# D-Hank/NeRF-tiny

Hardware: AMD Instinct MI355X
Metric: rays/sec (64 coarse + 128 fine samples), lego 400x400 (higher is better)
Workload: dtype f32

## Files before the change

### nerf-tiny_amd/csrc/field_fwd_reg.hip

```cpp
#include "field_common.h"
#include <type_traits>

namespace nerf {

constexpr int RM = 32;

template <int I0, int I1, class F>
__device__ __forceinline__ void static_for(F&& f) {
  if constexpr (I0 < I1) {
    f(std::integral_constant<int, I0>{});
    static_for<I0 + 1, I1>(f);
  }
}

template <int NFT>
struct WStage {
  float4 w[NFT];
};

template <int KB, int NFT>
__device__ __forceinline__ void stage_load(const float4* __restrict__ seg_lane, int kb, WStage<NFT>& s) {
#pragma unroll
  for (int f = 0; f < NFT; ++f) s.w[f] = seg_lane[(size_t)(f * KB + kb) * 64];
}

__device__ __forceinline__ float relu1(float x) { return __int_as_float(max(__float_as_int(x), 0)); }

__device__ __forceinline__ float f4c(const float4& v, int c) { return c == 0 ? v.x : (c == 1 ? v.y : (c == 2 ? v.z : v.w)); }

typedef int lds_i32 __attribute__((address_space(3), may_alias));
typedef int i32x4v __attribute__((ext_vector_type(4), may_alias));
typedef __attribute__((address_space(3))) i32x4v lds_i32x4;
constexpr int RELU_LDS_DWORDS = 2 * 4 * 64 * 4;
constexpr int COL_LDS_DWORDS = 3 * HALF + 4;
struct ReluLds {
  lds_i32* w;
  lds_i32* m[4];
};
__device__ __forceinline__ ReluLds relu_lds(lds_i32* base, int lane) {
  ReluLds L;
  L.w = base + 4 * lane;
#pragma unroll
  for (int c = 0; c < 4; ++c) L.m[c] = base + 4 * lane + ((c + (lane >> 3)) & 3);
  return L;
}
__device__ __forceinline__ float4 lds_ld4(const lds_i32* p) {
  const i32x4v v = *reinterpret_cast<const lds_i32x4*>(p);
  return make_float4(__int_as_float(v[0]), __int_as_float(v[1]), __int_as_float(v[2]), __int_as_float(v[3]));
}
template <typename DST>
__device__ __forceinline__ void relu_lds_op(const ReluLds& L, const f32x16& src, DST& dst, int dst0, int slot, int i) {
  const int g = i / 6, j = i - 6 * g, off = (slot * 4 + g) * 256;
  if (j == 0) {
    const i32x4v v = {__float_as_int(src[4 * g]), __float_as_int(src[4 * g + 1]), __float_as_int(src[4 * g + 2]), __float_as_int(src[4 * g + 3])};
    *reinterpret_cast<lds_i32x4*>(L.w + off) = v;
  } else if (j < 5) {
    __hip_atomic_fetch_max(L.m[j - 1] + off, 0, __ATOMIC_RELAXED, __HIP_MEMORY_SCOPE_WORKGROUP);
  } else {
    const i32x4v v = *reinterpret_cast<lds_i32x4*>(L.w + off);
#pragma unroll
    for (int c = 0; c < 4; ++c) dst[dst0 + c] = __int_as_float(v[c]);
  }
}

struct SaveIn {
  float* rows;
  uint16_t* mask;
};

__device__ __forceinline__ void bias_group(const float* b4h, int t, int g, f32x16& acc) {
  const float4 q = *reinterpret_cast<const float4*>(b4h + 32 * t + 8 * g);
  acc[4 * g + 0] = q.x;
  acc[4 * g + 1] = q.y;
  acc[4 * g + 2] = q.z;
  acc[4 * g + 3] = q.w;
}

template <int KB, int NFT, int NKB, int NNFT, bool ZERO_INIT, bool RELU_IN, int SAVE = 0, bool LDS_RELU = false, bool NEXT_RELU = false, int NEXT_BIAS = 0>
__device__ __forceinline__ void reg_layer(const int seg, const int next_seg , int lane,
                                          const f32x16* prev, f32x16* acc, WStage<8>& st0, const float* bv,
                                          const SaveIn sv, const RegBuf& rb, const ReluLds& rl, f32x4v& head,
                                          const float* nb = nullptr, f32x16* nacc = nullptr) {
  static_assert(!(LDS_RELU || NEXT_RELU || NEXT_BIAS) || SAVE != 1, "the saving forward keeps the VALU ReLU and the bias MFMAs");
  static_assert(NEXT_BIAS == 0 || ((LDS_RELU && RELU_IN) || NEXT_RELU), "the bias loads live in the stream with compile-time k-blocks");
  static_assert(NEXT_BIAS != 1 || (KB == 32 && RELU_IN), "NEXT_BIAS = 1 overwrites the 8 input tiles of a 256-wide ReLU layer");
  static_assert(NEXT_BIAS != 2 || KB == 8, "NEXT_BIAS = 2: one tile per k-block of layer 0");
  constexpr int KT = KB / 4;
  constexpr bool LR = LDS_RELU && RELU_IN;
  WStage<8> st1;
  const f32x16 zero = {0.f, 0.f, 0.f, 0.f, 0.f, 0.f, 0.f, 0.f, 0.f, 0.f, 0.f, 0.f, 0.f, 0.f, 0.f, 0.f};
  if (bv != nullptr) {
    const float one_h0 = (lane < 32) ? 1.0f : 0.0f;
#pragma unroll
    for (int f = 0; f < NFT; ++f) acc[f] = __builtin_amdgcn_mfma_f32_32x32x2f32(bv[f], one_h0, zero, 0, 0, 0);
  }
  f32x16 tin[2];
  if constexpr (LR) {
#pragma unroll
    for (int c = 0; c < 4; ++c) tin[0][c] = head[c];
    if (bv != nullptr) {
#pragma unroll
      for (int i = 6; i < 14; ++i) relu_lds_op(rl, prev[0], tin[0], 4 * (i / 6), 0, i);
#pragma unroll
      for (int i = 6; i < 14; ++i) {
        __builtin_amdgcn_sched_group_barrier(0x008, 1, 0);
        __builtin_amdgcn_sched_group_barrier(0x080, 1, 0);
      }
    }
  }
  [[maybe_unused]] const int lr0 = (bv != nullptr) ? 14 : 6;
  auto mask_word = [&](int t) {
    unsigned bits = 0;
#pragma unroll
    for (int r = 0; r < 16; ++r) bits |= (prev[t][r] > 0.f) ? (1u << r) : 0u;
    sv.mask[((t & 1) * 2) * 256 + (t >> 1) * 64] = (uint16_t)bits;
  };
  auto activate = [&](int t) {
    if constexpr (LR) {
      if (SAVE != 0) mask_word(t);
      return;
    }
#pragma unroll
    for (int r = 0; r < 16; ++r) tin[t & 1][r] = RELU_IN ? (SAVE == 1 ? fmaxf(prev[t][r], 0.f) : relu1(prev[t][r])) : prev[t][r];
#pragma unroll
    for (int r = 0; r < 16; ++r) asm volatile("" : "+v"(tin[t & 1][r]));
    if (SAVE == 1 || (SAVE == 2 && !RELU_IN)) {
#pragma unroll
      for (int g = 0; g < 4; ++g)
        store_row4(sv.rows + 32 * t + 8 * g, make_float4(tin[t & 1][4 * g], tin[t & 1][4 * g + 1], tin[t & 1][4 * g + 2], tin[t & 1][4 * g + 3]));
    }
    if (SAVE != 0 && RELU_IN) {
      unsigned bits = 0;
#pragma unroll
      for (int r = 0; r < 16; ++r) bits |= (prev[t][r] > 0.f) ? (1u << r) : 0u;
      sv.mask[((t & 1) * 2) * 256 + (t >> 1) * 64] = (uint16_t)bits;
    }
  };
  activate(0);
  if constexpr (!(LR || NEXT_RELU)) {
#pragma unroll
  for (int kb = 0; kb < KB; ++kb) {
    WStage<8>& ld = (kb & 1) ? st0 : st1;
    const WStage<8>& cur = (kb & 1) ? st1 : st0;
    if (kb + 1 < KB) {
#pragma unroll
      for (int f = 0; f < NFT; ++f) ld.w[f] = reg_ldw(rb, seg + (f * KB + kb + 1) * 64);
    } else if (next_seg >= 0) {
#pragma unroll
      for (int f = 0; f < NNFT; ++f) ld.w[f] = reg_ldw(rb, next_seg + (f * NKB) * 64);
    }
    __builtin_amdgcn_sched_barrier(0);
    if ((kb & 3) == 2 && (kb >> 2) + 1 < KT) activate((kb >> 2) + 1);
#pragma unroll
    for (int s = 0; s < 4; ++s) {
      const float b = tin[(kb >> 2) & 1][4 * (kb & 3) + s];
#pragma unroll
      for (int f = 0; f < NFT; ++f) {
        if (ZERO_INIT && bv == nullptr && kb == 0 && s == 0)
          acc[f] = __builtin_amdgcn_mfma_f32_32x32x2f32(f4c(cur.w[f], s), b, zero, 0, 0, 0);
        else
          acc[f] = __builtin_amdgcn_mfma_f32_32x32x2f32(f4c(cur.w[f], s), b, acc[f], 0, 0, 0);
      }
    }
  }
  } else {
  auto ds0 = [&](int kt, int k4, int s, int f) { const int i = lr0 + (k4 * 4 + s) * NFT + f; return (LR && kt == 0 && i < 24) ? i : -1; };
  auto ds1 = [&](int kt, int k4, int s, int f) { const int i = (k4 * 4 + s) * NFT + f - (NFT == 8 ? 64 : 16); return (LR && kt + 1 < KT && i >= 0 && i < 24) ? i : -1; };
  auto ds2 = [&](int kt, int k4, int s, int f) { return (NEXT_RELU && kt == KT - 1 && k4 == 3 && s == 3 && f < 6) ? f : -1; };
  auto nbt = [&](int kb, int s, int f) {
    if (NEXT_BIAS == 0 || s != 0 || f >= 4) return -1;
    if (NEXT_BIAS == 2) return kb;
    return kb == 1 ? 0 : (((kb & 3) == 3 && (kb >> 2) + 1 < KT) ? (kb >> 2) + 1 : -1);
  };
  static_for<0, KB>([&](auto kbc) __attribute__((always_inline)) {
    constexpr int kb = decltype(kbc)::value, kt = kb >> 2, k4 = kb & 3;
    WStage<8>& ld = (kb & 1) ? st0 : st1;
    const WStage<8>& cur = (kb & 1) ? st1 : st0;
    if (kb + 1 < KB) {
#pragma unroll
      for (int f = 0; f < NFT; ++f) ld.w[f] = reg_ldw(rb, seg + (f * KB + kb + 1) * 64);
    } else if (next_seg >= 0) {
#pragma unroll
      for (int f = 0; f < NNFT; ++f) ld.w[f] = reg_ldw(rb, next_seg + (f * NKB) * 64);
    }
    __builtin_amdgcn_sched_barrier(0);
    if (k4 == 2 && kt + 1 < KT) activate(kt + 1);
    bool any = false;
#pragma unroll
    for (int s = 0; s < 4; ++s) {
      const float b = tin[kt & 1][4 * k4 + s];
#pragma unroll
      for (int f = 0; f < NFT; ++f) {
        if (ZERO_INIT && bv == nullptr && kb == 0 && s == 0)
          acc[f] = __builtin_amdgcn_mfma_f32_32x32x2f32(f4c(cur.w[f], s), b, zero, 0, 0, 0);
        else
          acc[f] = __builtin_amdgcn_mfma_f32_32x32x2f32(f4c(cur.w[f], s), b, acc[f], 0, 0, 0);
        const int i0 = ds0(kt, k4, s, f), i1 = ds1(kt, k4, s, f), i2 = ds2(kt, k4, s, f);
        if constexpr (LR) {
          if (i0 >= 0) relu_lds_op(rl, prev[0], tin[0], 4 * (i0 / 6), 0, i0);
          if (i1 >= 0) relu_lds_op(rl, prev[kt + 1], tin[(kt + 1) & 1], 4 * (i1 / 6), (kt + 1) & 1, i1);
        }
        if constexpr (NEXT_RELU) {
          if (i2 >= 0) relu_lds_op(rl, acc[0], head, 0, 0, i2);
        }
        if constexpr (NEXT_BIAS != 0) {
          const int tb = nbt(kb, s, f);
          if (tb >= 0) bias_group(nb, tb, f, nacc[tb]);
          any |= tb >= 0;
        }
        any |= i0 >= 0 || i1 >= 0 || i2 >= 0;
      }
    }
    if (any) {
#pragma unroll
      for (int s = 0; s < 4; ++s)
#pragma unroll
        for (int f = 0; f < NFT; ++f) {
          const int n = (ds0(kt, k4, s, f) >= 0) + (ds1(kt, k4, s, f) >= 0) + (ds2(kt, k4, s, f) >= 0);
          __builtin_amdgcn_sched_group_barrier(0x008, 1, 0);
          if (n == 1) __builtin_amdgcn_sched_group_barrier(0x080, 1, 0);
          if (n == 2) __builtin_amdgcn_sched_group_barrier(0x080, 2, 0);
          if (nbt(kb, s, f) >= 0) __builtin_amdgcn_sched_group_barrier(0x020, 1, 0);
        }
    }
  });
  }
  if (KB & 1) st0 = st1;
}

template <int NFT>
__device__ __forceinline__ void bias_load(const float* __restrict__ bias, int lane, float (&bv)[8]) {
#pragma unroll
  for (int f = 0; f < NFT; ++f) bv[f] = bias[f * 32 + (lane & 31)];
}

#ifdef NERF_STAMPS
#define RSTAMP(slot)                                            \
  do {                                                          \
    __builtin_amdgcn_sched_barrier(0);                          \
    const unsigned long long t_ = __builtin_readcyclecounter(); \
    __builtin_amdgcn_sched_barrier(0);                          \
    tsum[slot] += t_ - tlast;                                   \
    tlast = t_;                                                 \
  } while (0)
#else
#define RSTAMP(slot) do { } while (0)
#endif

enum { SRC_RAYS = 0, SRC_POINTS = 1, SRC_LATTICE = 2, SRC_CORNERS = 3, SRC_BLOCKS = 4 };

template <bool SAVE, bool DEBUG, int SRC = SRC_RAYS, bool RGB = true, bool GSAVE = false>
__global__ __launch_bounds__(64, 1) void k_field_fwd_reg(const FieldArgs a, const QuerySrc q) {
#ifdef NERF_STAMPS
  unsigned long long tsum[12] = {0, 0, 0, 0, 0, 0, 0, 0, 0, 0, 0, 0};
  unsigned long long tlast = __builtin_readcyclecounter();
#endif
  const int lane = threadIdx.x, j = lane & 31, h = lane >> 5;
  const int m0 = blockIdx.x * RM;
  const int m = m0 + j;
  const bool valid = m < a.M;
  const int mc = valid ? m : a.M - 1;
  const int ray = (SRC == SRC_RAYS) ? mc / a.N : mc;
  const float* rf = (SRC == SRC_RAYS) ? a.rayf + (size_t)ray * RAYF : nullptr;
  const float4* wp = a.wp;
  const RegBuf rb = reg_buf(a.wp, threadIdx.x);

  WStage<8> st0;
  stage_load<8, 8>(wp + seg_off4(SEG_L0) + lane, 0, st0);
  constexpr bool LR = !SAVE;
  constexpr bool COL_LDS = LR && RGB;
  [[maybe_unused]] float4 cw0, cw1;
  [[maybe_unused]] float cb;
  if constexpr (COL_LDS) {
    const float4* wc4 = reinterpret_cast<const float4*>(a.w.p[W_COLOR]);
    cw0 = wc4[lane];
    cw1 = wc4[64 + j];
    cb = a.w.p[B_COLOR][lane < 3 ? lane : 2];
  }

  float p[3];
  [[maybe_unused]] bool band_keep = false;
  [[maybe_unused]] size_t band_at = 0;
  if constexpr (SRC == SRC_RAYS) {
    sample_point(rf, a.t[mc], p);
  } else if constexpr (SRC == SRC_POINTS) {
#pragma unroll
    for (int c = 0; c < 3; ++c) p[c] = q.points[(size_t)mc * 3 + c];
  } else if constexpr (SRC == SRC_LATTICE) {
    const int iz = mc % q.nz, ixy = mc / q.nz;
    const int iy = ixy % q.ny, ix = ixy / q.ny;
    p[0] = q.lo[0] + (float)ix * q.step[0];
    p[1] = q.lo[1] + (float)iy * q.step[1];
    p[2] = q.lo[2] + (float)iz * q.step[2];
  } else {
    static_assert(!RGB && !SAVE && !GSAVE && !DEBUG, "the band forms are sigma-only inference");
    const unsigned n[3] = {(unsigned)q.nx, (unsigned)q.ny, (unsigned)q.nz};
    unsigned idx[3];
    band_keep = valid;
    if constexpr (SRC == SRC_CORNERS) {
      const unsigned uz = (unsigned)mc % (unsigned)q.ext[2], uxy = (unsigned)mc / (unsigned)q.ext[2];
      idx[0] = uxy / (unsigned)q.ext[1] * (unsigned)q.r;
      idx[1] = uxy % (unsigned)q.ext[1] * (unsigned)q.r;
      idx[2] = uz * (unsigned)q.r;
    } else {
      const unsigned vol = (unsigned)(q.ext[0] * q.ext[1] * q.ext[2]);
      const unsigned e = (unsigned)mc / vol, l = (unsigned)mc - e * vol;
      band_keep = band_keep && (long long)q.e0 + e < *q.nlist;
      const unsigned b = band_keep ? (unsigned)q.list[(size_t)q.e0 + e] : 0u;
      const unsigned lz = l % (unsigned)q.ext[2], lxy = l / (unsigned)q.ext[2];
      const unsigned bz = b % (unsigned)q.nbz, bxy = b / (unsigned)q.nbz;
      idx[0] = bxy / (unsigned)q.nby * (unsigned)q.r + lxy / (unsigned)q.ext[1];
      idx[1] = bxy % (unsigned)q.nby * (unsigned)q.r + lxy % (unsigned)q.ext[1];
      idx[2] = bz * (unsigned)q.r + lz;
      band_keep = band_keep && idx[0] < n[0] && idx[1] < n[1] && idx[2] < n[2];
    }
#pragma unroll
    for (int c = 0; c < 3; ++c) idx[c] = idx[c] < n[c] ? idx[c] : n[c] - 1u;
    band_at = ((size_t)idx[0] * n[1] + idx[1]) * n[2] + idx[2];
    p[0] = q.lo[0] + (float)(int)idx[0] * q.step[0];
    p[1] = q.lo[1] + (float)(int)idx[1] * q.step[1];
    p[2] = q.lo[2] + (float)(int)idx[2] * q.step[2];
  }
  if (DEBUG && a.pts_dbg && valid && h == 0) {
    a.pts_dbg[(size_t)m * 3 + 0] = p[0];
    a.pts_dbg[(size_t)m * 3 + 1] = p[1];
    a.pts_dbg[(size_t)m * 3 + 2] = p[2];
  }
  f32x16 gp[2];
  static_for<0, 16>([&](auto ic) __attribute__((always_inline)) {
    constexpr int g8 = decltype(ic)::value >> 1, e = decltype(ic)::value & 1;
    constexpr int pa = 4 * g8 + e, pb = pa + 2;
    constexpr bool pad = pb >= 30;
    constexpr int ca = pa / 10, la = pa - 10 * ca, cb = pad ? ca : pb / 10, lb = pad ? la : pb - 10 * cb;
    static_assert(pa < 30, "lane half 0 never pads");
    constexpr uint32_t fa = kFreqPointLit[la], fb = kFreqPointLit[lb];
    const float x = (ca == cb) ? p[ca] : (h ? p[cb] : p[ca]);
    const float f = (la == lb) ? __uint_as_float(fa) : (h ? __uint_as_float(fb) : __uint_as_float(fa));
    float sv, cv;
    sincos_phase(x * f, sv, cv);
    if (pad) {
      sv = h ? 0.f : sv;
      cv = h ? 0.f : cv;
    }
    gp[g8 >> 2][4 * (g8 & 3) + 2 * e] = sv;
    gp[g8 >> 2][4 * (g8 & 3) + 2 * e + 1] = cv;
  });
  if (DEBUG && a.gp_dbg && valid) {
#pragma unroll
    for (int g8 = 0; g8 < 8; ++g8)
#pragma unroll
      for (int s = 0; s < 4; ++s) {
        const int k = 8 * g8 + 4 * h + s;
        if (k < POINT_DIM) a.gp_dbg[(size_t)m * POINT_DIM + k] = gp[g8 >> 2][4 * (g8 & 3) + s];
      }
  }

  const size_t MS = (size_t)a.MSrows * WIDTH;
  const long long rrow = valid ? (long long)(a.row0 + m) : a.Mtot + j;
  float* const srow = SAVE ? a.save + (size_t)rrow * WIDTH + 4 * h : nullptr;
  uint16_t* const mrow = (SAVE || GSAVE) ? a.masks + ((size_t)(a.tile0 + (m0 >> 6)) * 4 + ((m0 >> 5) & 1)) * 256 + h * 32 + j : nullptr;
  const size_t MKS = (size_t)a.tiles_tot * 4 * 256;
  auto sv_rows = [&](int tensor) { return SaveIn{SAVE ? srow + (size_t)tensor * MS : nullptr, nullptr}; };
  auto sv_relu = [&](int layer) { return SaveIn{SAVE ? srow + (size_t)layer * MS : nullptr, SAVE ? mrow + (size_t)layer * MKS : nullptr}; };
  float* const gprow = GSAVE ? a.save + (size_t)rrow * QGRAD_GP + 4 * h : nullptr;
  float* const crow = GSAVE ? a.save + (size_t)a.MSrows * QGRAD_GP + (size_t)rrow * QGRAD_C + 4 * h : nullptr;
  constexpr int SV = SAVE ? 1 : (GSAVE ? 2 : 0);
  auto sv_in = [&](int layer) { return GSAVE ? SaveIn{nullptr, mrow + (size_t)layer * MKS} : sv_relu(layer); };

  ReluLds rl{};
  [[maybe_unused]] lds_i32* col = nullptr;
  if constexpr (LR) {
    __shared__ int relu_slots[RELU_LDS_DWORDS + (COL_LDS ? COL_LDS_DWORDS : 0)];
    rl = relu_lds((lds_i32*)relu_slots, lane);
    if constexpr (COL_LDS) {
      col = (lds_i32*)relu_slots + RELU_LDS_DWORDS;
      const i32x4v v0 = {__float_as_int(cw0.x), __float_as_int(cw0.y), __float_as_int(cw0.z), __float_as_int(cw0.w)};
      const i32x4v v1 = {__float_as_int(cw1.x), __float_as_int(cw1.y), __float_as_int(cw1.z), __float_as_int(cw1.w)};
      *reinterpret_cast<lds_i32x4*>(col + 4 * lane) = v0;
      *reinterpret_cast<lds_i32x4*>(col + 4 * (64 + j)) = v1;
      col[3 * HALF + (lane < 3 ? lane : 2)] = __float_as_int(cb);
    }
  }
  f32x4v head = {0.f, 0.f, 0.f, 0.f};
  RSTAMP(0);
  f32x16 A[8], B[8];
  constexpr int L256 = 8 * 32 * 64;
  constexpr int sL1 = seg_off4(SEG_L1);
  constexpr int sL5 = seg_off4(SEG_L5);
  float bv[8];
  constexpr bool BL = LR;
  constexpr int NB1 = BL ? 1 : 0;
  auto bl = [&](int i) { return BL ? a.w.p[i] + 4 * h : nullptr; };
  auto bias_mfma = [&](int i) -> const float* {
    if constexpr (BL) return nullptr;
    bias_load<8>(a.w.p[i], lane, bv);
    return bv;
  };
  if constexpr (BL) {
#pragma unroll
    for (int t = 0; t < 8; ++t)
#pragma unroll
      for (int g = 0; g < 4; ++g) bias_group(bl(B_L0), t, g, A[t]);
  }

  reg_layer<8, 8, 32, 8, !BL, false, SV, LR, LR, BL ? 2 : 0>(seg_off4(SEG_L0), sL1, lane, gp, A, st0, bias_mfma(B_L0), GSAVE ? SaveIn{gprow, nullptr} : sv_rows(S_GP), rb, rl, head, bl(3), B);
  RSTAMP(1);
  reg_layer<32, 8, 32, 8, !BL, true, SV, LR, LR, NB1>(sL1, sL1 + L256, lane, A, B, st0, bias_mfma(3), sv_in(0), rb, rl, head, bl(5), A);
  reg_layer<32, 8, 32, 8, !BL, true, SV, LR, LR, NB1>(sL1 + L256, sL1 + 2 * L256, lane, B, A, st0, bias_mfma(5), sv_in(1), rb, rl, head, bl(7), B);
  reg_layer<32, 8, 32, 8, !BL, true, SV, LR, LR, NB1>(sL1 + 2 * L256, seg_off4(SEG_L4A), lane, A, B, st0, bias_mfma(7), sv_in(2), rb, rl, head, bl(9), A);
  RSTAMP(2);
  reg_layer<32, 8, 8, 8, !BL, true, SV, LR, false, NB1>(seg_off4(SEG_L4A), seg_off4(SEG_L4B), lane, B, A, st0, bias_mfma(9), sv_in(3), rb, rl, head, bl(11), B);
  reg_layer<8, 8, 32, 8, false, false, 0, LR, LR>(seg_off4(SEG_L4B), sL5, lane, gp, A, st0, nullptr, SaveIn{nullptr, nullptr}, rb, rl, head);
  RSTAMP(3);
  reg_layer<32, 8, 32, 8, !BL, true, SV, LR, LR, NB1>(sL5, sL5 + L256, lane, A, B, st0, bias_mfma(11), sv_in(4), rb, rl, head, bl(13), A);
  reg_layer<32, 8, 32, 8, !BL, true, SV, LR, LR, NB1>(sL5 + L256, sL5 + 2 * L256, lane, B, A, st0, bias_mfma(13), sv_in(5), rb, rl, head, bl(15), B);
  reg_layer<32, 8, 32, 4, !BL, true, SV, LR, false>(sL5 + 2 * L256, RGB ? seg_off4(SEG_FOLD) : -1, lane, A, B, st0, bias_mfma(15), sv_in(6), rb, rl, head);
  RSTAMP(4);
  {
    const float* ws = a.w.p[W_SIGMA] + 4 * h;
    float s = 0.f;
    float4 wq[2][4];
#pragma unroll
    for (int g = 0; g < 4; ++g) wq[0][g] = *reinterpret_cast<const float4*>(ws + 8 * g);
#pragma unroll
    for (int t = 0; t < 8; ++t) {
      if (t + 1 < 8) {
#pragma unroll
        for (int g = 0; g < 4; ++g) wq[(t + 1) & 1][g] = *reinterpret_cast<const float4*>(ws + 32 * (t + 1) + 8 * g);
      }
      if (SAVE) __builtin_amdgcn_sched_barrier(0);
      if (GSAVE) {
        unsigned bits = 0;
#pragma unroll
        for (int r = 0; r < 16; ++r) bits |= (B[t][r] > 0.f) ? (1u << r) : 0u;
        mrow[7 * MKS + ((t & 1) * 2) * 256 + (t >> 1) * 64] = (uint16_t)bits;
      }
#pragma unroll
      for (int g = 0; g < 4; ++g) {
        const float4 q = wq[t & 1][g];
        s = __builtin_fmaf(relu1(B[t][4 * g + 0]), q.x, s);
        s = __builtin_fmaf(relu1(B[t][4 * g + 1]), q.y, s);
        s = __builtin_fmaf(relu1(B[t][4 * g + 2]), q.z, s);
        s = __builtin_fmaf(relu1(B[t][4 * g + 3]), q.w, s);
      }
      if (SAVE) __builtin_amdgcn_sched_barrier(0);
    }
    s += __shfl_xor(s, 32);
    if constexpr (SRC == SRC_CORNERS || SRC == SRC_BLOCKS) {
      if (band_keep && h == 0) a.sigma[band_at] = fabsf(s + a.w.p[B_SIGMA][0]);
    } else if (valid && h == 0) {
      const float pre = s + a.w.p[B_SIGMA][0];
      a.sigma[m] = fabsf(pre);
      if (SAVE || GSAVE) a.spre[a.row0 + m] = pre;
    }
  }
  RSTAMP(5);
  if constexpr (!RGB) return;
  {
    const float* dv = a.dvec + (size_t)ray * HALF + 4 * h;
#pragma unroll
    for (int f = 0; f < 4; ++f)
#pragma unroll
      for (int g = 0; g < 4; ++g) {
        const float4 q = *reinterpret_cast<const float4*>(dv + 32 * f + 8 * g);
        A[f][4 * g + 0] = q.x;
        A[f][4 * g + 1] = q.y;
        A[f][4 * g + 2] = q.z;
        A[f][4 * g + 3] = q.w;
      }
  }
  reg_layer<32, 4, 32, 4, false, true, SAVE, false, false>(seg_off4(SEG_FOLD), -1, lane, B, A, st0, nullptr, GSAVE ? SaveIn{nullptr, nullptr} : sv_relu(7), rb, rl, head);
  RSTAMP(6);
  {
    const float* wc = a.w.p[W_COLOR] + 4 * h;
    float z0 = 0.f, z1 = 0.f, z2 = 0.f;
#pragma unroll
    for (int t = 0; t < 4; ++t)
#pragma unroll
      for (int g = 0; g < 4; ++g) {
        float4 q0, q1, q2;
        if constexpr (COL_LDS) {
          q0 = lds_ld4(col + 4 * h + 32 * t + 8 * g);
          q1 = lds_ld4(col + 4 * h + HALF + 32 * t + 8 * g);
          q2 = lds_ld4(col + 4 * h + 2 * HALF + 32 * t + 8 * g);
        } else {
          q0 = *reinterpret_cast<const float4*>(wc + 32 * t + 8 * g);
          q1 = *reinterpret_cast<const float4*>(wc + HALF + 32 * t + 8 * g);
          q2 = *reinterpret_cast<const float4*>(wc + 2 * HALF + 32 * t + 8 * g);
        }
        const float c0 = relu1(A[t][4 * g + 0]), c1 = relu1(A[t][4 * g + 1]);
        const float c2 = relu1(A[t][4 * g + 2]), c3 = relu1(A[t][4 * g + 3]);
        if (SAVE) store_row4(srow + S_C * MS + 32 * t + 8 * g, make_float4(c0, c1, c2, c3));
        if (GSAVE) store_row4(crow + 32 * t + 8 * g, make_float4(c0, c1, c2, c3));
        z0 = __builtin_fmaf(c3, q0.w, __builtin_fmaf(c2, q0.z, __builtin_fmaf(c1, q0.y, __builtin_fmaf(c0, q0.x, z0))));
        z1 = __builtin_fmaf(c3, q1.w, __builtin_fmaf(c2, q1.z, __builtin_fmaf(c1, q1.y, __builtin_fmaf(c0, q1.x, z1))));
        z2 = __builtin_fmaf(c3, q2.w, __builtin_fmaf(c2, q2.z, __builtin_fmaf(c1, q2.y, __builtin_fmaf(c0, q2.x, z2))));
      }
    z0 += __shfl_xor(z0, 32);
    z1 += __shfl_xor(z1, 32);
    z2 += __shfl_xor(z2, 32);
    float bc[3];
    if constexpr (COL_LDS) {
      const float4 b = lds_ld4(col + 3 * HALF);
      bc[0] = b.x, bc[1] = b.y, bc[2] = b.z;
    }
    if (valid && h == 0) {
      if constexpr (!COL_LDS) {
#pragma unroll
        for (int c = 0; c < 3; ++c) bc[c] = a.w.p[B_COLOR][c];
      }
      a.rgb[(size_t)m * 3 + 0] = 1.0f / (1.0f + expf(-(z0 + bc[0])));
      a.rgb[(size_t)m * 3 + 1] = 1.0f / (1.0f + expf(-(z1 + bc[1])));
      a.rgb[(size_t)m * 3 + 2] = 1.0f / (1.0f + expf(-(z2 + bc[2])));
    }
  }
#ifdef NERF_STAMPS
  RSTAMP(7);
  if (a.stamps && lane == 0) {
    for (int i = 0; i < 8; ++i) atomicAdd(a.stamps + i, tsum[i]);
    atomicAdd(a.stamps + 31, 1ull);
  }
#endif
}

hipError_t launch_field_fwd_reg(const FieldArgs& a, bool save, hipStream_t st) {
  const int tiles = (a.M + RM - 1) / RM;
  if (save)
    hipLaunchKernelGGL((k_field_fwd_reg<true, false>), dim3(tiles), dim3(64), 0, st, a, QuerySrc{});
  else if (a.pts_dbg || a.gp_dbg)
    hipLaunchKernelGGL((k_field_fwd_reg<false, true>), dim3(tiles), dim3(64), 0, st, a, QuerySrc{});
  else
    hipLaunchKernelGGL((k_field_fwd_reg<false, false>), dim3(tiles), dim3(64), 0, st, a, QuerySrc{});
  return hipGetLastError();
}

hipError_t launch_query_grad_fwd(const FieldArgs& a, const QuerySrc& q, bool rgb, hipStream_t st) {
  if (a.M <= 0) return hipSuccess;
  const unsigned tiles = (unsigned)(((long long)a.M + RM - 1) / RM);
  if (rgb)
    hipLaunchKernelGGL((k_field_fwd_reg<false, false, SRC_POINTS, true, true>), dim3(tiles), dim3(64), 0, st, a, q);
  else
    hipLaunchKernelGGL((k_field_fwd_reg<false, false, SRC_POINTS, false, true>), dim3(tiles), dim3(64), 0, st, a, q);
  return hipGetLastError();
}

hipError_t launch_query_reg(const FieldArgs& a, const QuerySrc& q, bool rgb, hipStream_t st) {
  if (a.M <= 0) return hipSuccess;
  const unsigned tiles = (unsigned)(((long long)a.M + RM - 1) / RM);
  if (q.points == nullptr)
    hipLaunchKernelGGL((k_field_fwd_reg<false, false, SRC_LATTICE, false>), dim3(tiles), dim3(64), 0, st, a, q);
  else if (rgb)
    hipLaunchKernelGGL((k_field_fwd_reg<false, false, SRC_POINTS, true>), dim3(tiles), dim3(64), 0, st, a, q);
  else
    hipLaunchKernelGGL((k_field_fwd_reg<false, false, SRC_POINTS, false>), dim3(tiles), dim3(64), 0, st, a, q);
  return hipGetLastError();
}

hipError_t launch_band_corners(const FieldArgs& a, const QuerySrc& q, hipStream_t st) {
  if (a.M <= 0) return hipSuccess;
  hipLaunchKernelGGL((k_field_fwd_reg<false, false, SRC_CORNERS, false>), dim3((unsigned)(((long long)a.M + RM - 1) / RM)), dim3(64), 0, st, a, q);
  return hipGetLastError();
}

hipError_t launch_band_blocks(const FieldArgs& a, const QuerySrc& q, hipStream_t st) {
  if (a.M <= 0) return hipSuccess;
  hipLaunchKernelGGL((k_field_fwd_reg<false, false, SRC_BLOCKS, false>), dim3((unsigned)(((long long)a.M + RM - 1) / RM)), dim3(64), 0, st, a, q);
  return hipGetLastError();
}

}
```

Baseline: 734,200.

## Shorten padded positional-encoding k-block and stage sigma weights in LDS

For the non-saving forward, the last k-block of the 8-wide input layers now runs 2 MFMA steps instead of 4. It uses the unpadded sin/cos values gathered during encoding and loads the weights at a per-lane offset, so multiplies against zero padding are skipped. The sigma head weights and bias are loaded once into LDS instead of being streamed from global memory per tile. Stamp-only timing records are also added under a debug macro. The risk is that the remapped weight offsets must exactly match the padded layout, and the extra LDS use could lower occupancy.

```diff
diff --git a/nerf-tiny_amd/csrc/field_fwd_reg.hip b/nerf-tiny_amd/csrc/field_fwd_reg.hip
--- a/nerf-tiny_amd/csrc/field_fwd_reg.hip
+++ b/nerf-tiny_amd/csrc/field_fwd_reg.hip
@@ -26,6 +26,13 @@
 
 __device__ __forceinline__ float relu1(float x) { return __int_as_float(max(__float_as_int(x), 0)); }
 
+__device__ __forceinline__ float4 reg_ldw_at(const RegBuf& rb, int lane_off, int f4) {
+  int soff = __builtin_amdgcn_readfirstlane(f4 * 16);
+  asm("" : "+s"(soff));
+  const rb_u32x4 v = __builtin_amdgcn_raw_buffer_load_b128(rb.rsrc, lane_off, soff, 0);
+  return make_float4(__uint_as_float(v.x), __uint_as_float(v.y), __uint_as_float(v.z), __uint_as_float(v.w));
+}
+
 __device__ __forceinline__ float f4c(const float4& v, int c) { return c == 0 ? v.x : (c == 1 ? v.y : (c == 2 ? v.z : v.w)); }
 
 typedef int lds_i32 __attribute__((address_space(3), may_alias));
@@ -33,6 +40,7 @@
 typedef __attribute__((address_space(3))) i32x4v lds_i32x4;
 constexpr int RELU_LDS_DWORDS = 2 * 4 * 64 * 4;
 constexpr int COL_LDS_DWORDS = 3 * HALF + 4;
+constexpr int SIG_LDS_DWORDS = WIDTH + 4;
 struct ReluLds {
   lds_i32* w;
   lds_i32* m[4];
@@ -76,11 +84,13 @@
   acc[4 * g + 3] = q.w;
 }
 
-template <int KB, int NFT, int NKB, int NNFT, bool ZERO_INIT, bool RELU_IN, int SAVE = 0, bool LDS_RELU = false, bool NEXT_RELU = false, int NEXT_BIAS = 0>
+template <int KB, int NFT, int NKB, int NNFT, bool ZERO_INIT, bool RELU_IN, int SAVE = 0, bool LDS_RELU = false, bool NEXT_RELU = false, int NEXT_BIAS = 0,
+          bool SHORT_K = false>
 __device__ __forceinline__ void reg_layer(const int seg, const int next_seg , int lane,
                                           const f32x16* prev, f32x16* acc, WStage<8>& st0, const float* bv,
                                           const SaveIn sv, const RegBuf& rb, const ReluLds& rl, f32x4v& head,
-                                          const float* nb = nullptr, f32x16* nacc = nullptr) {
+                                          const float* nb = nullptr, f32x16* nacc = nullptr, const float* bs = nullptr, int lo16 = 0) {
+  static_assert(!SHORT_K || (KB == 8 && !RELU_IN && SAVE != 1 && NEXT_RELU), "the short k-block lives in the stream with compile-time k-blocks");
   static_assert(!(LDS_RELU || NEXT_RELU || NEXT_BIAS) || SAVE != 1, "the saving forward keeps the VALU ReLU and the bias MFMAs");
   static_assert(NEXT_BIAS == 0 || ((LDS_RELU && RELU_IN) || NEXT_RELU), "the bias loads live in the stream with compile-time k-blocks");
   static_assert(NEXT_BIAS != 1 || (KB == 32 && RELU_IN), "NEXT_BIAS = 1 overwrites the 8 input tiles of a 256-wide ReLU layer");
@@ -120,14 +130,19 @@
       if (SAVE != 0) mask_word(t);
       return;
     }
-#pragma unroll
-    for (int r = 0; r < 16; ++r) tin[t & 1][r] = RELU_IN ? (SAVE == 1 ? fmaxf(prev[t][r], 0.f) : relu1(prev[t][r])) : prev[t][r];
-#pragma unroll
-    for (int r = 0; r < 16; ++r) asm volatile("" : "+v"(tin[t & 1][r]));
+    const int nr = (SHORT_K && t == KT - 1) ? 12 : 16;
+#pragma unroll
+    for (int r = 0; r < nr; ++r) tin[t & 1][r] = RELU_IN ? (SAVE == 1 ? fmaxf(prev[t][r], 0.f) : relu1(prev[t][r])) : prev[t][r];
+#pragma unroll
+    for (int r = 0; r < nr; ++r) asm volatile("" : "+v"(tin[t & 1][r]));
     if (SAVE == 1 || (SAVE == 2 && !RELU_IN)) {
 #pragma unroll
-      for (int g = 0; g < 4; ++g)
-        store_row4(sv.rows + 32 * t + 8 * g, make_float4(tin[t & 1][4 * g], tin[t & 1][4 * g + 1], tin[t & 1][4 * g + 2], tin[t & 1][4 * g + 3]));
+      for (int g = 0; g < 4; ++g) {
+        if (4 * g < nr)
+          store_row4(sv.rows + 32 * t + 8 * g, make_float4(tin[t & 1][4 * g], tin[t & 1][4 * g + 1], tin[t & 1][4 * g + 2], tin[t & 1][4 * g + 3]));
+        else
+          store_row4(sv.rows + 32 * t + 8 * g, make_float4(prev[t][4 * g], prev[t][4 * g + 1], prev[t][4 * g + 2], prev[t][4 * g + 3]));
+      }
     }
     if (SAVE != 0 && RELU_IN) {
       unsigned bits = 0;
@@ -166,7 +181,7 @@
   } else {
   auto ds0 = [&](int kt, int k4, int s, int f) { const int i = lr0 + (k4 * 4 + s) * NFT + f; return (LR && kt == 0 && i < 24) ? i : -1; };
   auto ds1 = [&](int kt, int k4, int s, int f) { const int i = (k4 * 4 + s) * NFT + f - (NFT == 8 ? 64 : 16); return (LR && kt + 1 < KT && i >= 0 && i < 24) ? i : -1; };
-  auto ds2 = [&](int kt, int k4, int s, int f) { return (NEXT_RELU && kt == KT - 1 && k4 == 3 && s == 3 && f < 6) ? f : -1; };
+  auto ds2 = [&](int kt, int k4, int s, int f) { return (NEXT_RELU && kt == KT - 1 && k4 == 3 && s == (SHORT_K ? 1 : 3) && f < 6) ? f : -1; };
   auto nbt = [&](int kb, int s, int f) {
     if (NEXT_BIAS == 0 || s != 0 || f >= 4) return -1;
     if (NEXT_BIAS == 2) return kb;
@@ -174,11 +189,13 @@
   };
   static_for<0, KB>([&](auto kbc) __attribute__((always_inline)) {
     constexpr int kb = decltype(kbc)::value, kt = kb >> 2, k4 = kb & 3;
+    constexpr bool SB = SHORT_K && kb == KB - 1;
+    constexpr int NS = SB ? 2 : 4;
     WStage<8>& ld = (kb & 1) ? st0 : st1;
     const WStage<8>& cur = (kb & 1) ? st1 : st0;
     if (kb + 1 < KB) {
 #pragma unroll
-      for (int f = 0; f < NFT; ++f) ld.w[f] = reg_ldw(rb, seg + (f * KB + kb + 1) * 64);
+      for (int f = 0; f < NFT; ++f) ld.w[f] = (SHORT_K && kb + 2 == KB) ? reg_ldw_at(rb, lo16, seg + (f * KB + kb + 1) * 64) : reg_ldw(rb, seg + (f * KB + kb + 1) * 64);
     } else if (next_seg >= 0) {
 #pragma unroll
       for (int f = 0; f < NNFT; ++f) ld.w[f] = reg_ldw(rb, next_seg + (f * NKB) * 64);
@@ -187,14 +204,15 @@
     if (k4 == 2 && kt + 1 < KT) activate(kt + 1);
     bool any = false;
 #pragma unroll
-    for (int s = 0; s < 4; ++s) {
-      const float b = tin[kt & 1][4 * k4 + s];
+    for (int s = 0; s < NS; ++s) {
+      const float b = SB ? bs[s] : tin[kt & 1][4 * k4 + s];
+      const int c = SB ? 2 * s : s;
 #pragma unroll
       for (int f = 0; f < NFT; ++f) {
         if (ZERO_INIT && bv == nullptr && kb == 0 && s == 0)
-          acc[f] = __builtin_amdgcn_mfma_f32_32x32x2f32(f4c(cur.w[f], s), b, zero, 0, 0, 0);
+          acc[f] = __builtin_amdgcn_mfma_f32_32x32x2f32(f4c(cur.w[f], c), b, zero, 0, 0, 0);
         else
-          acc[f] = __builtin_amdgcn_mfma_f32_32x32x2f32(f4c(cur.w[f], s), b, acc[f], 0, 0, 0);
+          acc[f] = __builtin_amdgcn_mfma_f32_32x32x2f32(f4c(cur.w[f], c), b, acc[f], 0, 0, 0);
         const int i0 = ds0(kt, k4, s, f), i1 = ds1(kt, k4, s, f), i2 = ds2(kt, k4, s, f);
         if constexpr (LR) {
           if (i0 >= 0) relu_lds_op(rl, prev[0], tin[0], 4 * (i0 / 6), 0, i0);
@@ -213,7 +231,7 @@
     }
     if (any) {
 #pragma unroll
-      for (int s = 0; s < 4; ++s)
+      for (int s = 0; s < NS; ++s)
 #pragma unroll
         for (int f = 0; f < NFT; ++f) {
           const int n = (ds0(kt, k4, s, f) >= 0) + (ds1(kt, k4, s, f) >= 0) + (ds2(kt, k4, s, f) >= 0);
@@ -243,6 +261,8 @@
     tsum[slot] += t_ - tlast;                                   \
     tlast = t_;                                                 \
   } while (0)
+constexpr int STAMP_CLK_AT = 1024, STAMP_CLK_N = 4096;
+static_assert(STAMP_CLK_AT + 2 * STAMP_CLK_N <= DBG_WORDS, "clock records inside the diagnostic area");
 #else
 #define RSTAMP(slot) do { } while (0)
 #endif
@@ -254,6 +274,7 @@
 #ifdef NERF_STAMPS
   unsigned long long tsum[12] = {0, 0, 0, 0, 0, 0, 0, 0, 0, 0, 0, 0};
   unsigned long long tlast = __builtin_readcyclecounter();
+  const unsigned long long tfirst = tlast, rfirst = __builtin_amdgcn_s_memrealtime();
 #endif
   const int lane = threadIdx.x, j = lane & 31, h = lane >> 5;
   const int m0 = blockIdx.x * RM;
@@ -276,6 +297,13 @@
     cw0 = wc4[lane];
     cw1 = wc4[64 + j];
     cb = a.w.p[B_COLOR][lane < 3 ? lane : 2];
+  }
+  constexpr bool SIG_LDS = LR;
+  [[maybe_unused]] float4 sw;
+  [[maybe_unused]] float sb;
+  if constexpr (SIG_LDS) {
+    sw = reinterpret_cast<const float4*>(a.w.p[W_SIGMA])[lane];
+    sb = a.w.p[B_SIGMA][0];
   }
 
   float p[3];
@@ -326,6 +354,9 @@
     a.pts_dbg[(size_t)m * 3 + 1] = p[1];
     a.pts_dbg[(size_t)m * 3 + 2] = p[2];
   }
+  constexpr bool SHORT_K = !SAVE;
+  [[maybe_unused]] float bs[2] = {0.f, 0.f};
+  [[maybe_unused]] const int lo16 = h ? rb.lane16 - 32 * 16 + 4 : rb.lane16;
   f32x16 gp[2];
   static_for<0, 16>([&](auto ic) __attribute__((always_inline)) {
     constexpr int g8 = decltype(ic)::value >> 1, e = decltype(ic)::value & 1;
@@ -339,6 +370,7 @@
     float sv, cv;
     sincos_phase(x * f, sv, cv);
     if (pad) {
+      if constexpr (SHORT_K) bs[e] = h ? cv : sv;
       sv = h ? 0.f : sv;
       cv = h ? 0.f : cv;
     }
@@ -369,8 +401,9 @@
 
   ReluLds rl{};
   [[maybe_unused]] lds_i32* col = nullptr;
+  [[maybe_unused]] lds_i32* sig = nullptr;
   if constexpr (LR) {
-    __shared__ int relu_slots[RELU_LDS_DWORDS + (COL_LDS ? COL_LDS_DWORDS : 0)];
+    __shared__ int relu_slots[RELU_LDS_DWORDS + (COL_LDS ? COL_LDS_DWORDS : 0) + (SIG_LDS ? SIG_LDS_DWORDS : 0)];
     rl = relu_lds((lds_i32*)relu_slots, lane);
     if constexpr (COL_LDS) {
       col = (lds_i32*)relu_slots + RELU_LDS_DWORDS;
@@ -379,6 +412,12 @@
       *reinterpret_cast<lds_i32x4*>(col + 4 * lane) = v0;
       *reinterpret_cast<lds_i32x4*>(col + 4 * (64 + j)) = v1;
       col[3 * HALF + (lane < 3 ? lane : 2)] = __float_as_int(cb);
+    }
+    if constexpr (SIG_LDS) {
+      sig = (lds_i32*)relu_slots + RELU_LDS_DWORDS + (COL_LDS ? COL_LDS_DWORDS : 0);
+      const i32x4v v = {__float_as_int(sw.x), __float_as_int(sw.y), __float_as_int(sw.z), __float_as_int(sw.w)};
+      *reinterpret_cast<lds_i32x4*>(sig + 4 * lane) = v;
+      sig[WIDTH] = __float_as_int(sb);
     }
   }
   f32x4v head = {0.f, 0.f, 0.f, 0.f};
@@ -403,14 +442,14 @@
       for (int g = 0; g < 4; ++g) bias_group(bl(B_L0), t, g, A[t]);
   }
 
-  reg_layer<8, 8, 32, 8, !BL, false, SV, LR, LR, BL ? 2 : 0>(seg_off4(SEG_L0), sL1, lane, gp, A, st0, bias_mfma(B_L0), GSAVE ? SaveIn{gprow, nullptr} : sv_rows(S_GP), rb, rl, head, bl(3), B);
+  reg_layer<8, 8, 32, 8, !BL, false, SV, LR, LR, BL ? 2 : 0, SHORT_K>(seg_off4(SEG_L0), sL1, lane, gp, A, st0, bias_mfma(B_L0), GSAVE ? SaveIn{gprow, nullptr} : sv_rows(S_GP), rb, rl, head, bl(3), B, bs, lo16);
   RSTAMP(1);
   reg_layer<32, 8, 32, 8, !BL, true, SV, LR, LR, NB1>(sL1, sL1 + L256, lane, A, B, st0, bias_mfma(3), sv_in(0), rb, rl, head, bl(5), A);
   reg_layer<32, 8, 32, 8, !BL, true, SV, LR, LR, NB1>(sL1 + L256, sL1 + 2 * L256, lane, B, A, st0, bias_mfma(5), sv_in(1), rb, rl, head, bl(7), B);
   reg_layer<32, 8, 32, 8, !BL, true, SV, LR, LR, NB1>(sL1 + 2 * L256, seg_off4(SEG_L4A), lane, A, B, st0, bias_mfma(7), sv_in(2), rb, rl, head, bl(9), A);
   RSTAMP(2);
   reg_layer<32, 8, 8, 8, !BL, true, SV, LR, false, NB1>(seg_off4(SEG_L4A), seg_off4(SEG_L4B), lane, B, A, st0, bias_mfma(9), sv_in(3), rb, rl, head, bl(11), B);
-  reg_layer<8, 8, 32, 8, false, false, 0, LR, LR>(seg_off4(SEG_L4B), sL5, lane, gp, A, st0, nullptr, SaveIn{nullptr, nullptr}, rb, rl, head);
+  reg_layer<8, 8, 32, 8, false, false, 0, LR, LR, 0, SHORT_K>(seg_off4(SEG_L4B), sL5, lane, gp, A, st0, nullptr, SaveIn{nullptr, nullptr}, rb, rl, head, nullptr, nullptr, bs, lo16);
   RSTAMP(3);
   reg_layer<32, 8, 32, 8, !BL, true, SV, LR, LR, NB1>(sL5, sL5 + L256, lane, A, B, st0, bias_mfma(11), sv_in(4), rb, rl, head, bl(13), A);
   reg_layer<32, 8, 32, 8, !BL, true, SV, LR, LR, NB1>(sL5 + L256, sL5 + 2 * L256, lane, B, A, st0, bias_mfma(13), sv_in(5), rb, rl, head, bl(15), B);
@@ -419,12 +458,14 @@
   {
     const float* ws = a.w.p[W_SIGMA] + 4 * h;
     float s = 0.f;
-    float4 wq[2][4];
-#pragma unroll
-    for (int g = 0; g < 4; ++g) wq[0][g] = *reinterpret_cast<const float4*>(ws + 8 * g);
+    [[maybe_unused]] float4 wq[2][4];
+    if constexpr (!SIG_LDS) {
+#pragma unroll
+      for (int g = 0; g < 4; ++g) wq[0][g] = *reinterpret_cast<const float4*>(ws + 8 * g);
+    }
 #pragma unroll
     for (int t = 0; t < 8; ++t) {
-      if (t + 1 < 8) {
+      if (!SIG_LDS && t + 1 < 8) {
 #pragma unroll
         for (int g = 0; g < 4; ++g) wq[(t + 1) & 1][g] = *reinterpret_cast<const float4*>(ws + 32 * (t + 1) + 8 * g);
       }
@@ -437,7 +478,9 @@
       }
 #pragma unroll
       for (int g = 0; g < 4; ++g) {
-        const float4 q = wq[t & 1][g];
+        float4 q;
+        if constexpr (SIG_LDS) q = lds_ld4(sig + 4 * h + 32 * t + 8 * g);
+        else q = wq[t & 1][g];
         s = __builtin_fmaf(relu1(B[t][4 * g + 0]), q.x, s);
         s = __builtin_fmaf(relu1(B[t][4 * g + 1]), q.y, s);
         s = __builtin_fmaf(relu1(B[t][4 * g + 2]), q.z, s);
@@ -446,10 +489,12 @@
       if (SAVE) __builtin_amdgcn_sched_barrier(0);
     }
     s += __shfl_xor(s, 32);
+    [[maybe_unused]] float bsig;
+    if constexpr (SIG_LDS) bsig = lds_ld4(sig + WIDTH).x;
     if constexpr (SRC == SRC_CORNERS || SRC == SRC_BLOCKS) {
-      if (band_keep && h == 0) a.sigma[band_at] = fabsf(s + a.w.p[B_SIGMA][0]);
+      if (band_keep && h == 0) a.sigma[band_at] = fabsf(s + (SIG_LDS ? bsig : a.w.p[B_SIGMA][0]));
     } else if (valid && h == 0) {
-      const float pre = s + a.w.p[B_SIGMA][0];
+      const float pre = s + (SIG_LDS ? bsig : a.w.p[B_SIGMA][0]);
       a.sigma[m] = fabsf(pre);
       if (SAVE || GSAVE) a.spre[a.row0 + m] = pre;
     }
@@ -519,6 +564,9 @@
   if (a.stamps && lane == 0) {
     for (int i = 0; i < 8; ++i) atomicAdd(a.stamps + i, tsum[i]);
     atomicAdd(a.stamps + 31, 1ull);
+    unsigned long long* rec = a.stamps + STAMP_CLK_AT + 2 * (blockIdx.x % STAMP_CLK_N);
+    rec[0] = tlast - tfirst;
+    rec[1] = __builtin_amdgcn_s_memrealtime() - rfirst;
   }
 #endif
 }
```

Result: no change. 736,700 (median of 6 runs) (+0.3%).
